# snipsco/sda

Hardware: AMD Instinct MI355X
Metric: share-gen + clerk-sum elements/sec (mod q) (higher is better)
Workload: dtype u64

## Files before the change

include/sda_hip_debug.h:

```cpp
#ifndef SDA_HIP_DEBUG_H
#define SDA_HIP_DEBUG_H
#include <stddef.h>
#ifdef __cplusplus
extern "C" {
#endif
int  sda_debug_hooks_compiled_in(void);
int  sda_debug_set_knob(const char* name, long value);
void sda_debug_reset_knobs(void);
int  sda_debug_env_knobs_compiled_in(void);
const char* sda_debug_last_kernel(void);
const char* sda_debug_last_reveal_kernel(void);
int  sda_debug_stream_create(void** stream);
int  sda_debug_stream_destroy(void* stream);
int  sda_debug_stream_synchronize(void* stream);
int  sda_debug_mem_info(size_t* free_bytes, size_t* total_bytes);
int  sda_debug_poly1305_rows_dev(const unsigned char* keys, const unsigned char* d_msgs, size_t msg_slot,
                                 const unsigned long long* d_msg_bytes, size_t rows, size_t max_msg_bytes, unsigned char* tags);
struct sda_secret_masker;
int  sda_debug_secret_masker_mask_batch_seeded_dev(struct sda_secret_masker* m, const unsigned* seed_words, const long long* d_secrets,
                                                   size_t participants, size_t len, size_t secrets_stride,
                                                   unsigned long long first_participant, long long* d_masks, size_t mask_stride,
                                                   long long* d_masked, size_t masked_stride, void* stream);
int  sda_debug_last_mask_plan(unsigned out[4]);
struct sda_sharing_scheme;
int  sda_debug_select_path(const struct sda_sharing_scheme* scheme, const char* knobs, char* out, size_t cap);
#ifdef __cplusplus
}
#endif
#endif
```

sda_amd/capi.py:

```python
from __future__ import annotations

import ctypes as C
import os

_HERE = os.path.dirname(os.path.abspath(__file__))
RELEASE_LIB_PATH = os.path.join(_HERE, "lib", "libsda_hip.so")
TEST_LIB_PATH = os.path.join(_HERE, "lib", "libsda_hip_test.so")
LIB_PATH = os.environ.get("SDA_HIP_LIBRARY") or RELEASE_LIB_PATH

c_i64p = C.POINTER(C.c_int64)
c_u8p = C.POINTER(C.c_uint8)
c_sizep = C.POINTER(C.c_size_t)
c_i64pp = C.POINTER(c_i64p)
c_voidpp = C.POINTER(C.c_void_p)

OK = 0
ERR_BATCH_INPUT_WRONG_LENGTH = -1
ERR_SHARING_FAILED = -2
ERR_INPUTS_MUST_HAVE_SAME_LENGTH = -3
ERR_NOT_ENOUGH_SHARES = -4
ERR_WRONG_DIMENSION = -5
ERR_MISMATCHING_DIMENSION = -6
ERR_ASSERTION = -7
ERR_INVALID_ARGUMENT = -8
# ... 161 lines not shown
                                                    C.c_size_t, C.c_size_t, C.c_void_p, C.c_size_t, C.c_void_p, C.c_void_p]),
    "sda_share_generator_generate_sealed_rows_dev": (C.c_int, [_H, _H, _H, C.c_char_p, C.c_char_p, C.c_void_p, C.c_size_t, C.c_size_t,
                                                               C.c_size_t, C.c_uint64, C.c_void_p, C.c_size_t, C.c_void_p, C.c_void_p]),
    "sda_share_combiner_update_sealed_rows_dev": (C.c_int, [_H, _H, _H, C.c_char_p, C.c_char_p, C.c_void_p, C.c_size_t,
                                                            C.c_void_p, C.c_size_t, C.c_size_t, C.c_void_p, C.c_void_p,
                                                            C.c_void_p]),
    "sda_share_combiner_finish_sealed_rows_dev": (C.c_int, [_H, _H, _H, C.c_char_p, C.c_char_p, C.c_void_p, C.c_size_t, C.c_void_p,
                                                            C.c_void_p]),
    "sda_mask_combiner_begin_dev": (C.c_int, [_H, C.c_size_t, C.c_void_p]),
    "sda_mask_combiner_update_dev": (C.c_int, [_H, C.c_void_p, C.c_size_t, C.c_size_t, C.c_size_t, C.c_void_p]),
    "sda_mask_combiner_update_sealed_rows_dev": (C.c_int, [_H, _H, _H, C.c_char_p, C.c_char_p, C.c_void_p, C.c_size_t,
                                                           C.c_void_p, C.c_size_t, C.c_size_t, C.c_void_p, C.c_void_p,
                                                           C.c_void_p]),
    "sda_mask_combiner_finish_dev": (C.c_int, [_H, C.c_void_p, C.c_size_t, C.c_void_p]),
    "sda_secret_reconstructor_begin_dev": (C.c_int, [_H, c_sizep, C.c_size_t, C.c_size_t, C.c_void_p]),
    "sda_secret_reconstructor_update_dev": (C.c_int, [_H, C.c_size_t, C.c_void_p, C.c_size_t, C.c_size_t, C.c_void_p]),
    "sda_secret_reconstructor_update_sealed_rows_dev": (C.c_int, [_H, _H, _H, C.c_char_p, C.c_char_p, C.c_size_t, C.c_void_p,
                                                                  C.c_size_t, C.c_void_p, C.c_size_t, C.c_size_t, C.c_void_p,
                                                                  C.c_void_p, C.c_void_p]),
    "sda_secret_reconstructor_finish_dev": (C.c_int, [_H, C.c_void_p, C.c_size_t, C.c_void_p]),
    "sda_comm_unique_id": (C.c_int, [c_u8p]),
    "sda_comm_init": (C.c_int, [c_u8p, C.c_int, C.c_int, _HP]),
    "sda_comm_free": (None, [_H]),
    "sda_comm_rank": (C.c_int, [_H]),
    "sda_comm_world": (C.c_int, [_H]),
    "sda_comm_device": (C.c_int, [_H]),
    "sda_comm_rccl_version": (C.c_int, []),
    "sda_modular_allreduce_dev": (C.c_int, [_H, C.c_int64, C.c_void_p, C.c_size_t, C.c_void_p, C.c_void_p]),
    "sda_modsum_parts_dev": (C.c_int, [C.c_int64, C.c_void_p, C.c_size_t, C.c_size_t, C.c_size_t, C.c_void_p,
                                       C.c_void_p]),
    "sda_fill_synthetic_dev": (C.c_int, [C.c_void_p, C.c_size_t, C.c_size_t, C.c_size_t, C.c_uint64, C.c_uint64,
                                         C.c_int64, C.c_void_p]),
    "sda_event_create": (C.c_int, [c_voidpp]),
    "sda_event_destroy": (C.c_int, [C.c_void_p]),
    "sda_event_record": (C.c_int, [C.c_void_p, C.c_void_p]),
    "sda_event_elapsed_ms": (C.c_int, [C.c_void_p, C.c_void_p, C.POINTER(C.c_float)]),
}

HOOK_SIGNATURES = {
    "sda_debug_set_knob": (C.c_int, [C.c_char_p, C.c_long]),
    "sda_debug_reset_knobs": (None, []),
    "sda_debug_env_knobs_compiled_in": (C.c_int, []),
    "sda_debug_stream_create": (C.c_int, [c_voidpp]),
    "sda_debug_stream_destroy": (C.c_int, [C.c_void_p]),
    "sda_debug_stream_synchronize": (C.c_int, [C.c_void_p]),
    "sda_debug_mem_info": (C.c_int, [c_sizep, c_sizep]),
    "sda_debug_select_path": (C.c_int, [_SS, C.c_char_p, C.c_char_p, C.c_size_t]),
    "sda_debug_last_reveal_kernel": (C.c_char_p, []),
    "sda_debug_poly1305_rows_dev": (C.c_int, [C.c_char_p, C.c_void_p, C.c_size_t, C.c_void_p, C.c_size_t, C.c_size_t, C.c_char_p]),
    "sda_debug_secret_masker_mask_batch_seeded_dev": (C.c_int, [_H, C.c_void_p, C.c_void_p, C.c_size_t, C.c_size_t, C.c_size_t,
                                                                C.c_uint64, C.c_void_p, C.c_size_t, C.c_void_p, C.c_size_t,
                                                                C.c_void_p]),
    "sda_debug_last_mask_plan": (C.c_int, [C.POINTER(C.c_uint * 4)]),
}

_loaded = {}
_active_path = None


def _load_path(path):
    lib = _loaded.get(path)
    if lib is None:
        if not os.path.exists(path):
            raise OSError(f"{path} is missing: build it with __graft_entry__.build(); "
                          "there is no fallback implementation")
        lib = C.CDLL(path)
        for name, (res, args) in SIGNATURES.items():
            fn = getattr(lib, name)
            fn.restype = res
            fn.argtypes = args
        if lib.sda_debug_hooks_compiled_in():
            for name, (res, args) in HOOK_SIGNATURES.items():
                fn = getattr(lib, name)
                fn.restype = res
                fn.argtypes = args
        _loaded[path] = lib
    return lib


class _ActiveLibrary:

    def __getattr__(self, name):
        lib = _load_path(_active_path or LIB_PATH)
        if name in HOOK_SIGNATURES and not lib.sda_debug_hooks_compiled_in():
            raise AttributeError(f"{name} exists only in libsda_hip_test.so: call sda_amd.capi.use_test_hooks() first "
                                 f"(the release library {active_path()} has no test hooks)")
        return getattr(lib, name)


_proxy = _ActiveLibrary()


def load():
    _load_path(_active_path or LIB_PATH)
    return _proxy


def active_path() -> str:
    return _active_path or LIB_PATH


def has_test_hooks() -> bool:
    return bool(_load_path(active_path()).sda_debug_hooks_compiled_in())


def use_test_hooks():
# ... 43 lines not shown
```

sda_amd/csrc/kernels.hpp:

```cpp
#pragma once
#include <stddef.h>
#include <stdint.h>
#include <hip/hip_runtime_api.h>

namespace sda {

struct ModParams {
    uint64_t m;
    uint64_t mu;
    uint64_t lemire_thr;
    uint64_t lemire_thr2;
};

struct MontParams {
    uint64_t p;
    uint64_t pinv;
};

struct DrbgKey {
    uint32_t w[8];
};

#define SDA_MAT_ARG_MAX 448
struct MatArg {
// ... 196 lines not shown
size_t scan_aux_entries(size_t n);
hipError_t launch_scan_u32(const uint32_t* d_in, uint64_t* d_out, size_t n, uint64_t* d_total, uint64_t* d_aux,
                           hipStream_t s);
hipError_t launch_varint_write(const VarintRows& R, const uint64_t* d_block_off, uint8_t* d_out,
                               uint64_t* d_row_offsets, hipStream_t s);
hipError_t launch_varint_count(const uint8_t* d_bytes, size_t n_bytes, uint32_t* d_block_counts, hipStream_t s);
hipError_t launch_varint_decode(const uint8_t* d_bytes, size_t n_bytes, const uint64_t* d_block_val_off,
                                size_t rows, size_t len, size_t row_stride, int64_t* d_out, uint32_t* d_status,
                                hipStream_t s);
struct RowRanges {
    const uint64_t* offsets;
    const uint64_t* lengths;
    uint64_t slot;
};
hipError_t launch_varint_stream_decode(const uint8_t* d_bytes, size_t n_bytes, const RowRanges& rr, size_t rows,
                                       size_t len, size_t row_stride, int64_t* d_out, uint32_t* d_status, hipStream_t s);
hipError_t launch_varint_stream_encode(const VarintRows& R, uint8_t* d_out, size_t slot_bytes, uint64_t* d_row_bytes,
                                       hipStream_t s);
hipError_t launch_varint_stream_combine(const uint8_t* d_bytes, size_t n_bytes, const RowRanges& rr, size_t jobs,
                                        size_t rows_per_job, size_t len, uint64_t* d_acc_lo, int64_t* d_acc_hi,
                                        uint32_t* d_status, hipStream_t s);
struct SboxState;
hipError_t launch_sealed_stream_combine(const uint8_t* d_boxes, size_t slot, const uint64_t* d_row_bytes, size_t rows,
                                        size_t max_box_bytes, const SboxState* d_states, size_t len, uint64_t* d_acc_lo,
                                        int64_t* d_acc_hi, uint32_t* d_status, hipStream_t s, int* waves);
struct WeightedJob {
    const uint64_t* Rt;
    uint32_t k;
    uint64_t batches;
    uint64_t m, mu, pinv;
};
hipError_t launch_sealed_stream_weighted(const uint8_t* d_boxes, size_t slot, const uint64_t* d_row_bytes, size_t rows,
                                         size_t max_box_bytes, const SboxState* d_states, size_t len, size_t first_pos,
                                         const WeightedJob& J, uint64_t* d_acc_lo, int64_t* d_acc_hi, uint32_t* d_status,
                                         hipStream_t s);
hipError_t launch_weighted_rows(const int64_t* d_shares, size_t row_stride, size_t rows, size_t first_pos, const WeightedJob& J,
                                uint64_t* d_acc_lo, int64_t* d_acc_hi, hipStream_t s);
hipError_t launch_transpose_u64(const uint64_t* d_in, uint64_t* d_out, uint32_t k, uint32_t n, hipStream_t s);
hipError_t launch_varint_seal_stream(const VarintRows& R, uint8_t* d_boxes, size_t slot_bytes, const SboxState* d_states,
                                     uint64_t* d_msg_bytes, hipStream_t s);
struct ShareJob {
    const int64_t* secrets;  size_t secrets_stride;
    size_t len, participants;
    uint64_t batches;
    uint64_t first_participant;
    uint32_t n, k, t;
    uint32_t additive;
    uint32_t direct_rows;
    const uint64_t* M;
    ModParams mod;
    MontParams mont;
    DrbgKey key;
};
hipError_t launch_share_seal_stream(const ShareJob& J, int rounds, uint8_t* d_boxes, size_t slot_bytes, const SboxState* d_states,
                                    uint64_t* d_msg_bytes, hipStream_t s);
struct SumRows {
    const uint64_t* acc_lo;  const int64_t* acc_hi;
    size_t jobs, len;
    uint64_t m, mu;
};
size_t sum_seal_blocks(size_t len);
hipError_t launch_sum_lengths(const SumRows& S, uint32_t* d_block_bytes, hipStream_t s);
hipError_t launch_sum_seal_wide(const SumRows& S, const uint64_t* d_block_off, uint8_t* d_boxes, size_t slot_bytes,
                                const SboxState* d_states, uint64_t* d_msg_bytes, hipStream_t s);
hipError_t launch_varint_rowcheck(const uint8_t* d_bytes, size_t n_bytes, const uint64_t* d_offsets, size_t rows,
                                  size_t len, const uint64_t* d_block_val_off, uint32_t* d_status, hipStream_t s);

hipError_t launch_base64_decode_rows(const uint8_t* d_text, const uint64_t* d_offsets, size_t text_slot,
                                     const uint64_t* d_lengths, size_t rows, size_t max_chars, uint8_t* d_out,
                                     size_t out_slot, uint64_t* d_out_bytes, uint32_t* d_status, uint32_t* d_row_status,
                                     hipStream_t s);
hipError_t launch_base64_encode_rows(const uint8_t* d_in, size_t in_slot, const uint64_t* d_in_bytes, size_t rows,
                                     size_t max_bytes, uint8_t* d_text, size_t text_slot, uint64_t* d_text_bytes,
                                     hipStream_t s);

struct SboxState {
    uint32_t subkey[8];
    uint32_t n0, n1;
    uint32_t s[4];
    uint32_t r64[5], rS[5];
    uint32_t bad, pad[7];
    uint32_t rpow[64][5];
};
size_t sbox_regions(size_t max_msg_bytes);
hipError_t launch_sealedbox_open(const uint8_t pk[32], const uint8_t sk[32], const uint8_t* d_boxes, size_t slot,
                                 const uint64_t* d_row_bytes, size_t rows, size_t max_box_bytes, uint8_t* d_out, size_t out_slot,
                                 uint64_t* d_out_bytes, uint32_t* d_ok, uint32_t* d_status, SboxState* d_states,
                                 uint32_t* d_partial, hipStream_t s);
hipError_t launch_sealedbox_verify(const uint8_t pk[32], const uint8_t sk[32], const uint8_t* d_boxes, size_t slot,
                                   const uint64_t* d_row_bytes, size_t rows, size_t max_box_bytes, uint64_t* d_out_bytes,
                                   uint32_t* d_ok, uint32_t* d_status, SboxState* d_states, uint32_t* d_partial, hipStream_t s);
hipError_t launch_sealedbox_seal(const uint8_t* d_esk, const uint8_t* d_pks, size_t n_pks, size_t rows_per_key,
                                 const uint8_t* d_msgs, size_t msg_slot, const uint64_t* d_msg_bytes, size_t rows,
                                 size_t max_msg_bytes, uint8_t* d_boxes, size_t slot, uint64_t* d_row_bytes, SboxState* d_states,
                                 uint32_t* d_partial, hipStream_t s);
hipError_t launch_sealedbox_seal_setup(const uint8_t* d_esk, const uint8_t* d_pks, size_t n_pks, size_t rows_per_key, uint8_t* d_boxes,
                                       size_t slot, size_t rows, SboxState* d_states, hipStream_t s);
hipError_t launch_sealedbox_seal_auth(const uint64_t* d_msg_bytes, size_t rows, size_t max_msg_bytes, uint8_t* d_boxes, size_t slot,
                                      uint64_t* d_row_bytes, SboxState* d_states, uint32_t* d_partial, hipStream_t s);
hipError_t launch_sealedbox_poly_test(const uint8_t* d_keys, const uint8_t* d_msgs, size_t msg_slot, const uint64_t* d_msg_bytes,
                                      size_t rows, size_t max_msg_bytes, uint8_t* d_heads, uint64_t* d_head_bytes,
                                      SboxState* d_states, uint32_t* d_partial, hipStream_t s);

hipError_t launch_modsum_parts(const int64_t* d_parts, size_t parts, size_t part_stride, size_t len,
                               const ModParams& mod, int64_t* d_out, hipStream_t s);
hipError_t launch_fill_synthetic(int64_t* d_out, size_t participants, size_t len, size_t stride,
// ... 5 lines not shown
```

sda_amd/csrc/sda_capi.cpp:

```cpp
#include "../../include/sda_hip.h"

#include <hip/hip_runtime_api.h>
#include <errno.h>
#include <stdarg.h>
#include <stdio.h>
#include <stdlib.h>
#include <atomic>
#include <string.h>
#include <sys/random.h>

#include <algorithm>
#include <new>
#include <string>
#include <vector>

#include "capi_internal.hpp"
#include "host_chacha.hpp"
#include "host_math.hpp"
#include "kernels.hpp"
#include "modarith.hpp"
#include "path_select.hpp"

using namespace sda;

// ... 2540 lines not shown
    if (L == 0) HIP_TRY(launch_varint_stream_decode(d_bytes, rows * slot_bytes, rr, rows, 0, 0, nullptr, d_status, c->ctx.pick(stream)));
    return c->mark_pending(c->ctx.pick(stream));
}

extern "C" int sda_share_combiner_update_sealed_rows_dev(sda_share_combiner_t* c, sda_varint_codec_t* codec, sda_sealedbox_t* b,
                                                         const uint8_t pk[32], const uint8_t sk[32], const uint8_t* d_boxes,
                                                         size_t slot_bytes, const uint64_t* d_row_bytes, size_t rows,
                                                         size_t max_box_bytes, uint32_t* d_ok, uint32_t* d_status, void* stream) {
    if (!c || !codec || !b) return fail(SDA_ERR_INVALID_ARGUMENT, "NULL handle");
    if (!pk || !sk) return fail(SDA_ERR_INVALID_ARGUMENT, "NULL argument");
    if (!c->begun) return fail(SDA_ERR_STATE, "update before begin");
    if (c->acc.rust_signed) return fail(SDA_ERR_UNSUPPORTED, "the wire-fed updates sum in 128 bits: SDA_VALUES_RUST_SIGNED takes decode + update[_dev]");
    if (c->jobs != 1) return fail(SDA_ERR_STATE, "the sealed form feeds ONE job: the combiner was begun with %zu jobs", c->jobs);
    if (rows == 0) return SDA_OK;
    if (!d_status || !d_boxes || !d_row_bytes) return fail(SDA_ERR_INVALID_ARGUMENT, "NULL device pointer");
    if (slot_bytes % 16 || ((uintptr_t)d_boxes & 15u)) return fail(SDA_ERR_INVALID_ARGUMENT, "boxes must be 16-byte aligned (buffer and slot_bytes)");
    if (max_box_bytes > slot_bytes) return fail(SDA_ERR_INVALID_ARGUMENT, "max_box_bytes exceeds slot_bytes");
    SDA_TRY(c->ctx.use());
    hipStream_t s = c->ctx.pick(stream);
    const SboxState* d_states = nullptr;
    SDA_TRY(capi_sealedbox_verify_rows(b, pk, sk, d_boxes, slot_bytes, d_row_bytes, rows, max_box_bytes, d_ok, d_status, c->ctx.device, s,
                                       &d_states));
    SDA_TRY(c->join_pending(s));
    int waves = 0;
    HIP_TRY(launch_sealed_stream_combine(d_boxes, slot_bytes, d_row_bytes, rows, max_box_bytes, d_states, c->dimension,
                                         c->acc.lo.as<uint64_t>(), c->acc.hi.as<int64_t>(), d_status, s, &waves));
    note_kernel("sbox_poly_kernel + sealed_stream_combine_kernel<%d>", waves);
    snprintf(g_last_call_kernels, sizeof g_last_call_kernels, "%s", g_last_gen_kernel);
    return c->mark_pending(s);
}

extern "C" int sda_sealedbox_seal_share_rows_dev(sda_sealedbox_t* b, sda_varint_codec_t* codec, const uint8_t* pks, size_t n_pks,
                                                 size_t rows_per_key, const uint8_t* esk, const int64_t* d_values, size_t rows,
                                                 size_t len, size_t row_stride, uint8_t* d_boxes, size_t slot_bytes,
                                                 uint64_t* d_row_bytes, void* stream) {
    if (!b || !codec) return fail(SDA_ERR_INVALID_ARGUMENT, "NULL handle");
    if (!pks || n_pks == 0 || rows_per_key == 0) return fail(SDA_ERR_INVALID_ARGUMENT, "bad recipient key arguments");
    if (!d_boxes || !d_row_bytes || (len > 0 && !d_values)) return fail(SDA_ERR_INVALID_ARGUMENT, "NULL device pointer");
    if (row_stride < len) return fail(SDA_ERR_INVALID_ARGUMENT, "row_stride < len");
    if (slot_bytes % 16 || ((uintptr_t)d_boxes & 15u)) return fail(SDA_ERR_INVALID_ARGUMENT, "boxes must be 16-byte aligned (buffer and slot_bytes)");
    if (len > (SIZE_MAX - 64) / 10 || slot_bytes < sda_varint_slot_size(len) + SDA_SEALBYTES)
        return fail(SDA_ERR_INVALID_ARGUMENT, "slot_bytes < sda_varint_slot_size(len) + 48");
    if (capi_sealedbox_device(b) != codec->ctx.device)
        return fail(SDA_ERR_INVALID_ARGUMENT, "the sealed-box handle lives on device %d, the codec on device %d", capi_sealedbox_device(b), codec->ctx.device);
    if (rows == 0) return SDA_OK;
    SDA_TRY(codec->ctx.use());
    SDA_TRY(capi_sealedbox_seal_share_rows(b, pks, n_pks, rows_per_key, esk, VarintRows{d_values, rows, len, row_stride}, d_boxes, slot_bytes,
                                           d_row_bytes, codec->ctx.pick(stream)));
    note_kernel("varint_seal_stream_kernel + sbox_poly_kernel");
    snprintf(g_last_call_kernels, sizeof g_last_call_kernels, "%s", g_last_gen_kernel);
    return SDA_OK;
}

extern "C" int sda_share_generator_generate_sealed_rows_dev(sda_share_generator_t* g, sda_varint_codec_t* codec, sda_sealedbox_t* b,
                                                            const uint8_t* pks, const uint8_t* esk, const int64_t* d_secrets,
                                                            size_t participants, size_t len, size_t secrets_stride,
                                                            uint64_t first_participant, uint8_t* d_boxes, size_t slot_bytes,
                                                            uint64_t* d_row_bytes, void* stream) {
    if (!g || !codec || !b) return fail(SDA_ERR_INVALID_ARGUMENT, "NULL handle");
    if (!pks) return fail(SDA_ERR_INVALID_ARGUMENT, "NULL clerk keys");
    if (!d_boxes || !d_row_bytes || (len > 0 && !d_secrets)) return fail(SDA_ERR_INVALID_ARGUMENT, "NULL device pointer");
    if (secrets_stride < len) return fail(SDA_ERR_INVALID_ARGUMENT, "secrets_stride < len");
    if (slot_bytes % 16 || ((uintptr_t)d_boxes & 15u)) return fail(SDA_ERR_INVALID_ARGUMENT, "boxes must be 16-byte aligned (buffer and slot_bytes)");
    const size_t B = (len + g->k - 1) / g->k;
    if (B > (SIZE_MAX - 64) / 10 || slot_bytes < sda_varint_slot_size(B) + SDA_SEALBYTES)
        return fail(SDA_ERR_INVALID_ARGUMENT, "slot_bytes < sda_varint_slot_size(batches) + 48");
    if (capi_sealedbox_device(b) != codec->ctx.device || g->ctx.device != codec->ctx.device)
        return fail(SDA_ERR_INVALID_ARGUMENT, "the generator lives on device %d, the sealed-box handle on device %d, the codec on device %d",
                    g->ctx.device, capi_sealedbox_device(b), codec->ctx.device);
    if (g->rust_signed)
        return fail(SDA_ERR_UNSUPPORTED, "the sealed form computes canonical shares only: SDA_VALUES_RUST_SIGNED takes generate_batch_dev + seal_share_rows_dev");
    if (!g->additive && g->k + g->t > 32)
        return fail(SDA_ERR_UNSUPPORTED, "the sealed form serves packed Shamir with secret_count + privacy_threshold <= 32 (this scheme: %u): "
                                         "call generate_batch_dev + sda_sealedbox_seal_share_rows_dev", g->k + g->t);
    size_t rows = 0;
    if (__builtin_mul_overflow(participants, (size_t)g->n, &rows)) return fail(SDA_ERR_INVALID_ARGUMENT, "participants * share_count overflows");
    if (participants == 0) return SDA_OK;
    SDA_TRY(check_streams(first_participant, participants));
    SDA_TRY(g->ctx.use());
    const bool sys = effective_sys(g);
    if (!g->additive && !g->mseal_loaded) {
        SDA_TRY(g->d_Mseal.reserve((g->Mmont.size() + g->Msys.size()) * 8));
        HIP_TRY(hipMemcpy(g->d_Mseal.p, g->Mmont.data(), g->Mmont.size() * 8, hipMemcpyHostToDevice));
        if (!g->Msys.empty())
            HIP_TRY(hipMemcpy(g->d_Mseal.as<uint64_t>() + g->Mmont.size(), g->Msys.data(), g->Msys.size() * 8, hipMemcpyHostToDevice));
        g->mseal_loaded = true;
    }
    ShareJob J{};
    J.secrets = d_secrets; J.secrets_stride = secrets_stride; J.len = len; J.participants = participants; J.batches = B;
    J.first_participant = first_participant;
    J.n = g->n; J.k = g->k; J.t = g->t; J.additive = g->additive ? 1u : 0u;
    J.direct_rows = sys ? g->t : 0;
    J.M = g->additive ? nullptr : g->d_Mseal.as<uint64_t>() + (sys ? g->Mmont.size() : 0);
    J.mod = g->mod; J.mont = g->mont;
    if (len > 0) J.key = g->drbg.call_key();
    g_last_gen_kernel[0] = 0;
    const int st = capi_sealedbox_seal_generated_rows(b, pks, esk, J, g->drbg.rounds, d_boxes, slot_bytes, d_row_bytes, g->ctx.pick(stream));
    explicit_bzero(&J.key, sizeof J.key);
    if (st != SDA_OK) return st;
    note_kernel("share_seal_stream_kernel<%d> + sbox_poly_kernel", g->drbg.rounds);
    snprintf(g_last_call_kernels, sizeof g_last_call_kernels, "%s", g_last_gen_kernel);
    return SDA_OK;
}

extern "C" int sda_share_combiner_finish_sealed_rows_dev(sda_share_combiner_t* c, sda_varint_codec_t* codec, sda_sealedbox_t* b,
                                                         const uint8_t pk[32], const uint8_t* esk, uint8_t* d_boxes, size_t slot_bytes,
// ... 108 lines not shown
```

sda_amd/csrc/varint_kernels.hip:

```cpp
#include <hip/hip_runtime.h>
#include <stdint.h>

#include "capi_internal.hpp"
#include "drbg_quad.hpp"
#include "kernels.hpp"
#include "modarith.hpp"
#include "sbox_primitives.hpp"

namespace sda {

static constexpr int kVT = 256;
static constexpr int kVals = 8;
static constexpr int kBytes = 16;

__device__ __forceinline__ uint64_t zigzag(int64_t v) { return ((uint64_t)v << 1) ^ (uint64_t)(v >> 63); }
__device__ __forceinline__ uint32_t varint_len(uint64_t zz) {
    const uint32_t x = (64u - (uint32_t)__clzll(zz | 1ull)) + 6u;
    return (x * 37u) >> 8;
}

__device__ __forceinline__ uint32_t block_exscan(uint32_t v, uint32_t* lds_waves, uint32_t* total) {
    const int lane = threadIdx.x & 63, wave = threadIdx.x >> 6;
    uint32_t incl = v;
#pragma unroll
// ... 986 lines not shown
            x = (int64_t)s0; y = (int64_t)s1;
            return;
        }
        U128 a0{0, 0}, a1{0, 0};
        uint32_t since = 0;
        const uint64_t e0 = b0 * J.k, e1 = e0 + J.k;
        for (uint32_t i = 0; i < J.k; ++i) {
            const uint64_t v0 = e0 + i < J.len ? canon_i64(sp[e0 + i], m, mu) : 0;
            const uint64_t v1 = e1 + i < J.len ? canon_i64(sp[e1 + i], m, mu) : 0;
            const uint64_t cf = row[i];
            mac128(a0, cf, v0);
            mac128(a1, cf, v1);
            if (++since == 4) { mont_acc_condsub(a0, J.mont.p); mont_acc_condsub(a1, J.mont.p); since = 0; }
        }
        for (uint32_t i = 0; i < T; ++i) {
            drbg_pair<ROUNDS>(J.key, qc, stream, pair, T, i, J.mod, r0, r1);
            const uint64_t cf = row[J.k + i];
            mac128(a0, cf, r0);
            mac128(a1, cf, r1);
            if (++since == 4) { mont_acc_condsub(a0, J.mont.p); mont_acc_condsub(a1, J.mont.p); since = 0; }
        }
        mont_acc_condsub(a0, J.mont.p);
        mont_acc_condsub(a1, J.mont.p);
        x = (int64_t)mont_redc(a0, J.mont.p, J.mont.pinv);
        y = (int64_t)mont_redc(a1, J.mont.p, J.mont.pinv);
    }
};

template <int ROUNDS>
__global__ __launch_bounds__(kStreamWaves * 64) void share_seal_stream_kernel(ShareJob J, uint32_t by_rows, uint8_t* __restrict__ boxes,
                                                                              uint64_t slot, const SboxState* __restrict__ states,
                                                                              uint64_t* __restrict__ msg_bytes) {
    __shared__ __attribute__((aligned(16))) uint8_t tiles[kStreamWaves][kEncTile];
    __shared__ uint32_t kstream[kStreamWaves][kKsTile];
    const int wave = __builtin_amdgcn_readfirstlane(threadIdx.x >> 6);
    uint64_t c, p;
    if (by_rows) {
        const uint64_t r = (uint64_t)blockIdx.x * kStreamWaves + wave;
        c = r / J.participants; p = r - c * J.participants;
    } else {
        const uint32_t groups = (J.n + kStreamWaves - 1) / kStreamWaves;
        p = blockIdx.x / groups;
        c = (uint64_t)(blockIdx.x - p * groups) * kStreamWaves + wave;
    }
    if (c >= J.n || p >= J.participants) return;
    const uint64_t r = c * J.participants + p;
    if (states[r].bad) { if ((threadIdx.x & 63) == 0) msg_bytes[r] = 0; return; }
    EncXSalsa crypt;
    crypt.open(states[r], kstream[wave]);
    ShareValues<ROUNDS> vals(J, (uint32_t)c, p);
    encode_row(vals, J.batches, r, boxes + r * slot + 48, tiles[wave], msg_bytes, crypt);
}

static constexpr int kSumVals = kVT * kVals;
static constexpr int kSumStage = 64 + kSumVals * 10;
static constexpr int kSumKsBlocks = kSumStage / 64;
static constexpr int kSumKsStride = 17;

size_t sum_seal_blocks(size_t len) { return (size_t)((len + kSumVals - 1) / kSumVals); }

__global__ __launch_bounds__(kVT) void sum_len_kernel(SumRows S, uint32_t* __restrict__ block_bytes) {
    __shared__ uint32_t waves[kVT / 64];
    const uint64_t job = blockIdx.y;
    const uint64_t* lo = S.acc_lo + job * S.len;
    const int64_t* hi = S.acc_hi + job * S.len;
    const uint64_t i0 = (uint64_t)blockIdx.x * kSumVals + threadIdx.x;
    uint32_t sum = 0;
    for (int u = 0; u < kVals; ++u) {
        const uint64_t i = i0 + (uint64_t)u * kVT;
        if (i < S.len) sum += varint_len(zigzag((int64_t)mod_i128(lo[i], hi[i], S.m, S.mu)));
    }
    uint32_t total;
    (void)block_exscan(sum, waves, &total);
    if (threadIdx.x == 0) block_bytes[job * gridDim.x + blockIdx.x] = total;
}

__global__ __launch_bounds__(kVT) void sum_seal_wide_kernel(SumRows S, const uint64_t* __restrict__ block_off, uint8_t* __restrict__ boxes,
                                                            uint64_t slot, const SboxState* __restrict__ states,
                                                            uint64_t* __restrict__ msg_bytes) {
    __shared__ uint32_t waves[kVT / 64];
    __shared__ __attribute__((aligned(16))) uint8_t stage[kSumStage + 16];
    __shared__ uint32_t ks[kSumKsBlocks * kSumKsStride];
    const uint64_t job = blockIdx.y, blk = blockIdx.x, n_blk = gridDim.x;
    const bool last = blk + 1 == n_blk;
    const SboxState& st = states[job];
    if (st.bad) { if (last && threadIdx.x == 0) msg_bytes[job] = 0; return; }
    const uint64_t off = block_off[job * n_blk + blk] - block_off[job * n_blk];
    const uint32_t pad = (uint32_t)((off + 32) & 63u);
    const uint64_t ks0 = (off + 32) >> 6;
    const uint64_t* lo = S.acc_lo + job * S.len;
    const int64_t* hi = S.acc_hi + job * S.len;
    const uint64_t i0 = blk * kSumVals + (uint64_t)threadIdx.x * kVals;
    uint64_t zz[kVals];
    uint32_t ln[kVals];
    uint32_t sum = 0;
    for (int k = 0; k < kVals; ++k) {
        zz[k] = 0; ln[k] = 0;
        if (i0 + k < S.len) {
            zz[k] = zigzag((int64_t)mod_i128(lo[i0 + k], hi[i0 + k], S.m, S.mu));
            ln[k] = varint_len(zz[k]);
            sum += ln[k];
        }
    }
    uint32_t total;
    uint32_t pos = pad + block_exscan(sum, waves, &total);
#pragma unroll
// ... 92 lines not shown
                                       size_t len, size_t row_stride, int64_t* d_out, uint32_t* d_status, hipStream_t s) {
    if (rows == 0) return hipSuccess;
    varint_stream_decode_kernel<<<dim3((unsigned)vceil(rows, kStreamWaves)), dim3(kStreamWaves * 64), 0, s>>>(
        d_bytes, n_bytes, d_offsets, rows, len, row_stride, d_out, d_status);
    return hipGetLastError();
}

hipError_t launch_varint_stream_encode(const VarintRows& R, uint8_t* d_out, size_t slot_bytes, uint64_t* d_row_bytes,
                                       hipStream_t s) {
    if (R.rows == 0) return hipSuccess;
    varint_stream_encode_kernel<<<dim3((unsigned)vceil(R.rows, kStreamWaves)), dim3(kStreamWaves * 64), residency_pad_bytes(knob(KNOB_WIRE_WG_PER_CU), 8192), s>>>(
        R, d_out, slot_bytes, d_row_bytes);
    return hipGetLastError();
}

hipError_t launch_varint_seal_stream(const VarintRows& R, uint8_t* d_boxes, size_t slot_bytes, const SboxState* d_states,
                                     uint64_t* d_msg_bytes, hipStream_t s) {
    if (R.rows == 0) return hipSuccess;
    const uint64_t groups = vceil(R.rows, kStreamWaves);
    if (groups > 0x7FFFFFFFull) return hipErrorInvalidConfiguration;
    varint_seal_stream_kernel<<<dim3((unsigned)groups), dim3(kStreamWaves * 64), 0, s>>>(R, d_boxes, slot_bytes, d_states, d_msg_bytes);
    return hipGetLastError();
}

static bool sum_grid(const SumRows& S, dim3* grid) {
    const uint64_t nb = sum_seal_blocks(S.len);
    if (S.jobs > 65535 || nb * S.jobs > 0xFFFFFFFFull / kVT) return false;
    *grid = dim3((unsigned)nb, (unsigned)S.jobs);
    return true;
}

hipError_t launch_sum_lengths(const SumRows& S, uint32_t* d_block_bytes, hipStream_t s) {
    if (S.jobs == 0 || S.len == 0) return hipSuccess;
    dim3 grid;
    if (!sum_grid(S, &grid)) return hipErrorInvalidConfiguration;
    sum_len_kernel<<<grid, dim3(kVT), 0, s>>>(S, d_block_bytes);
    return hipGetLastError();
}

hipError_t launch_sum_seal_wide(const SumRows& S, const uint64_t* d_block_off, uint8_t* d_boxes, size_t slot_bytes,
                                const SboxState* d_states, uint64_t* d_msg_bytes, hipStream_t s) {
    if (S.jobs == 0) return hipSuccess;
    if (S.len == 0) return hipMemsetAsync(d_msg_bytes, 0, S.jobs * sizeof(uint64_t), s);
    dim3 grid;
    if (!sum_grid(S, &grid)) return hipErrorInvalidConfiguration;
    sum_seal_wide_kernel<<<grid, dim3(kVT), 0, s>>>(S, d_block_off, d_boxes, slot_bytes, d_states, d_msg_bytes);
    return hipGetLastError();
}

hipError_t launch_share_seal_stream(const ShareJob& J, int rounds, uint8_t* d_boxes, size_t slot_bytes, const SboxState* d_states,
                                    uint64_t* d_msg_bytes, hipStream_t s) {
    if (J.participants == 0 || J.n == 0) return hipSuccess;
    const bool by_rows = knob(KNOB_GENSEAL_BY_ROWS) != 0;
    const uint64_t groups = by_rows ? vceil((uint64_t)J.n * J.participants, kStreamWaves) : vceil(J.n, kStreamWaves) * (uint64_t)J.participants;
    if (groups > 0x7FFFFFFFull) return hipErrorInvalidConfiguration;
    const dim3 grid((unsigned)groups), block(kStreamWaves * 64);
    switch (rounds) {
        case 20: share_seal_stream_kernel<20><<<grid, block, 0, s>>>(J, by_rows, d_boxes, slot_bytes, d_states, d_msg_bytes); break;
        case 12: share_seal_stream_kernel<12><<<grid, block, 0, s>>>(J, by_rows, d_boxes, slot_bytes, d_states, d_msg_bytes); break;
        case 8: share_seal_stream_kernel<8><<<grid, block, 0, s>>>(J, by_rows, d_boxes, slot_bytes, d_states, d_msg_bytes); break;
        default: return hipErrorInvalidValue;
    }
    return hipGetLastError();
}

hipError_t launch_varint_stream_combine(const uint8_t* d_bytes, size_t n_bytes, const RowRanges& d_offsets, size_t jobs,
                                        size_t rows_per_job, size_t len, uint64_t* d_acc_lo, int64_t* d_acc_hi,
                                        uint32_t* d_status, hipStream_t s) {
    if (jobs == 0 || rows_per_job == 0 || len == 0) return hipSuccess;
    const bool wide = vceil(rows_per_job, 16) * jobs >= 512;
    const uint64_t groups = vceil(rows_per_job, wide ? 16 : 8);
    if (groups * jobs > 0x7FFFFFFFull) return hipErrorInvalidConfiguration;
    if (wide)
        varint_stream_combine_kernel<16><<<dim3((unsigned)(groups * jobs)), dim3(16 * 64), residency_pad_bytes(knob(KNOB_WIRE_WG_PER_CU), 49152), s>>>(
            d_bytes, n_bytes, d_offsets, rows_per_job, groups, len, d_acc_lo, d_acc_hi, d_status);
    else
        varint_stream_combine_kernel<8><<<dim3((unsigned)(groups * jobs)), dim3(8 * 64), 0, s>>>(
            d_bytes, n_bytes, d_offsets, rows_per_job, groups, len, d_acc_lo, d_acc_hi, d_status);
    return hipGetLastError();
}

hipError_t launch_sealed_stream_combine(const uint8_t* d_boxes, size_t slot, const uint64_t* d_row_bytes, size_t rows,
                                        size_t max_box_bytes, const SboxState* d_states, size_t len, uint64_t* d_acc_lo,
                                        int64_t* d_acc_hi, uint32_t* d_status, hipStream_t s, int* waves) {
    if (waves) *waves = 0;
    if (rows == 0) return hipSuccess;
    const bool wide = knob(KNOB_SEALED_WAVES) == 16;
    const uint64_t groups = vceil(rows, wide ? 16 : 8);
    if (groups > 0x7FFFFFFFull) return hipErrorInvalidConfiguration;
    if (waves) *waves = wide ? 16 : 8;
    if (wide)
        sealed_stream_combine_kernel<16><<<dim3((unsigned)groups), dim3(16 * 64), 0, s>>>(d_boxes, slot, d_row_bytes, max_box_bytes, d_states,
                                                                                       rows, len, d_acc_lo, d_acc_hi, d_status);
    else
        sealed_stream_combine_kernel<8><<<dim3((unsigned)groups), dim3(8 * 64), 0, s>>>(d_boxes, slot, d_row_bytes, max_box_bytes, d_states,
                                                                                     rows, len, d_acc_lo, d_acc_hi, d_status);
    return hipGetLastError();
}

hipError_t launch_sealed_stream_weighted(const uint8_t* d_boxes, size_t slot, const uint64_t* d_row_bytes, size_t rows,
                                         size_t max_box_bytes, const SboxState* d_states, size_t len, size_t first_pos,
                                         const WeightedJob& J, uint64_t* d_acc_lo, int64_t* d_acc_hi, uint32_t* d_status,
                                         hipStream_t s) {
    if (rows == 0) return hipSuccess;
    const uint64_t groups = vceil(rows, 8);
    if (groups > 0x7FFFFFFFull) return hipErrorInvalidConfiguration;
// ... 41 lines not shown
```

Before: 118.4 billion.

## Share DRBG draws and secrets across clerk waves via LDS staging in share-seal kernel

Result: no change. 118.4 billion, median of 6 (+0.0%).

```diff
diff --git a/include/sda_hip_debug.h b/include/sda_hip_debug.h
--- a/include/sda_hip_debug.h
+++ b/include/sda_hip_debug.h
@@ -22,6 +22,7 @@
                                                    unsigned long long first_participant, long long* d_masks, size_t mask_stride,
                                                    long long* d_masked, size_t masked_stride, void* stream);
 int  sda_debug_last_mask_plan(unsigned out[4]);
+int  sda_debug_genseal_geometry(unsigned share_count, unsigned secret_count, unsigned privacy_threshold, int additive, unsigned out[6]);
 struct sda_sharing_scheme;
 int  sda_debug_select_path(const struct sda_sharing_scheme* scheme, const char* knobs, char* out, size_t cap);
 #ifdef __cplusplus
diff --git a/sda_amd/capi.py b/sda_amd/capi.py
--- a/sda_amd/capi.py
+++ b/sda_amd/capi.py
@@ -237,6 +237,7 @@
                                                                 C.c_uint64, C.c_void_p, C.c_size_t, C.c_void_p, C.c_size_t,
                                                                 C.c_void_p]),
     "sda_debug_last_mask_plan": (C.c_int, [C.POINTER(C.c_uint * 4)]),
+    "sda_debug_genseal_geometry": (C.c_int, [C.c_uint, C.c_uint, C.c_uint, C.c_int, C.POINTER(C.c_uint * 6)]),
 }
 
 _loaded = {}
diff --git a/sda_amd/csrc/kernels.hpp b/sda_amd/csrc/kernels.hpp
--- a/sda_amd/csrc/kernels.hpp
+++ b/sda_amd/csrc/kernels.hpp
@@ -272,6 +272,8 @@
     MontParams mont;
     DrbgKey key;
 };
+struct GensealGeometry { uint32_t shared, waves, groups, steps, terms, lds_bytes; };
+GensealGeometry genseal_geometry(uint32_t n, uint32_t kt, uint32_t additive);
 hipError_t launch_share_seal_stream(const ShareJob& J, int rounds, uint8_t* d_boxes, size_t slot_bytes, const SboxState* d_states,
                                     uint64_t* d_msg_bytes, hipStream_t s);
 struct SumRows {
diff --git a/sda_amd/csrc/sda_capi.cpp b/sda_amd/csrc/sda_capi.cpp
--- a/sda_amd/csrc/sda_capi.cpp
+++ b/sda_amd/csrc/sda_capi.cpp
@@ -2616,6 +2616,17 @@
     return SDA_OK;
 }
 
+#ifdef SDA_TEST_HOOKS
+extern "C" int sda_debug_genseal_geometry(unsigned share_count, unsigned secret_count, unsigned privacy_threshold, int additive,
+                                          unsigned out[6]) {
+    if (!out) return fail(SDA_ERR_INVALID_ARGUMENT, "out is NULL");
+    if (share_count == 0) return fail(SDA_ERR_INVALID_ARGUMENT, "share_count is 0");
+    const GensealGeometry G = genseal_geometry(share_count, secret_count + privacy_threshold, additive ? 1u : 0u);
+    out[0] = G.shared; out[1] = G.waves; out[2] = G.groups; out[3] = G.steps; out[4] = G.terms; out[5] = G.lds_bytes;
+    return SDA_OK;
+}
+#endif
+
 extern "C" int sda_share_generator_generate_sealed_rows_dev(sda_share_generator_t* g, sda_varint_codec_t* codec, sda_sealedbox_t* b,
                                                             const uint8_t* pks, const uint8_t* esk, const int64_t* d_secrets,
                                                             size_t participants, size_t len, size_t secrets_stride,
diff --git a/sda_amd/csrc/varint_kernels.hip b/sda_amd/csrc/varint_kernels.hip
--- a/sda_amd/csrc/varint_kernels.hip
+++ b/sda_amd/csrc/varint_kernels.hip
@@ -1062,6 +1062,161 @@
     encode_row(vals, J.batches, r, boxes + r * slot + 48, tiles[wave], msg_bytes, crypt);
 }
 
+static constexpr int kShareWaves = 8;
+static constexpr uint32_t kShareWaveLds = kEncTile + 4 * kKsTile;
+static constexpr uint32_t kShareLdsBudget = 80 * 1024;
+
+GensealGeometry genseal_geometry(uint32_t n, uint32_t kt, uint32_t additive) {
+    GensealGeometry g{};
+    if (n == 0) return g;
+    g.terms = additive ? n : kt;
+    g.groups = (n + kShareWaves - 1) / kShareWaves;
+    g.waves = (n + g.groups - 1) / g.groups;
+    const uint32_t left = kShareLdsBudget - g.waves * kShareWaveLds, step = g.terms * kEncVals * 8;
+    g.steps = step == 0 ? 0 : left / step < 8 ? left / step : 8;
+    g.lds_bytes = g.waves * kShareWaveLds + g.steps * step;
+    g.shared = g.steps >= 1;
+    return g;
+}
+
+template <int ROUNDS>
+struct SharedShareValues {
+    static constexpr int kDepth = 1;
+    const ShareJob& J;
+    const int64_t* __restrict__ sp;
+    const uint64_t* __restrict__ row;
+    uint64_t* stage;
+    uint64_t stream, n_steps;
+    uint32_t S, terms, units_per_step, first_draw, wave, waves, phase;
+    uint32_t T, own;
+    bool secret_last;
+    QuadCol qc;
+    __device__ __forceinline__ SharedShareValues(const ShareJob& J_, uint64_t* stage_, uint32_t S_, uint32_t terms_, uint32_t c0,
+                                                 uint32_t size, uint32_t c, uint64_t p, uint32_t wave_, uint32_t waves_)
+        : J(J_), stage(stage_), S(S_), terms(terms_), wave(wave_), waves(waves_), phase(0) {
+        sp = J.secrets + p * J.secrets_stride;
+        stream = J.first_participant + p;
+        qc = quad_col(J.key);
+        n_steps = (J.batches + kEncVals - 1) / kEncVals;
+        T = J.additive ? J.n - 1 : J.t;
+        const uint32_t direct = J.additive ? J.n - 1 : J.direct_rows;
+        row = J.additive || c < direct ? nullptr : J.M + (uint64_t)(c - direct) * (J.k + J.t);
+        if (J.additive) {
+            secret_last = c0 + size == J.n;
+            units_per_step = secret_last ? J.n : size;
+            first_draw = secret_last ? 0 : c0;
+            own = c < direct ? c - first_draw : terms;
+        } else {
+            secret_last = false;
+            units_per_step = J.k + J.t;
+            first_draw = 0;
+            own = c < direct ? J.k + c : terms;
+        }
+    }
+    __device__ __forceinline__ uint64_t* slot(uint32_t s, uint32_t term) const {
+        return stage + ((s * terms + term) * (uint32_t)kEncVals + 2u * (threadIdx.x & 63u));
+    }
+    __device__ __forceinline__ void begin_block(uint64_t j0) {
+        __syncthreads();
+        const uint64_t left = n_steps - j0;
+        const uint32_t steps = left < S ? (uint32_t)left : S;
+        const uint32_t units = steps * units_per_step;
+        const uint64_t m = J.mod.m, mu = J.mod.mu;
+        uint32_t s = 0, term = wave;
+        for (uint32_t u = wave; u < units; u += waves, term += waves) {
+            while (term >= units_per_step) { term -= units_per_step; ++s; }
+            const uint64_t pair = (j0 + s) * (kEncVals / 2) + (threadIdx.x & 63u);
+            const uint64_t b0 = 2 * pair;
+            uint64_t v0, v1;
+            if (J.additive) {
+                if (secret_last && term == J.n - 1) {
+                    v0 = b0 < J.len ? canon_i64(sp[b0], m, mu) : 0;
+                    v1 = b0 + 1 < J.len ? canon_i64(sp[b0 + 1], m, mu) : 0;
+                } else {
+                    drbg_pair<ROUNDS>(J.key, qc, stream, pair, T, first_draw + term, J.mod, v0, v1);
+                }
+            } else if (term < J.k) {
+                const uint64_t e0 = b0 * J.k + term, e1 = e0 + J.k;
+                v0 = e0 < J.len ? canon_i64(sp[e0], m, mu) : 0;
+                v1 = e1 < J.len ? canon_i64(sp[e1], m, mu) : 0;
+            } else {
+                drbg_pair<ROUNDS>(J.key, qc, stream, pair, T, term - J.k, J.mod, v0, v1);
+            }
+            uint64_t* q = slot(s, term);
+            q[0] = v0; q[1] = v1;
+        }
+        __syncthreads();
+    }
+    __device__ __forceinline__ void idle() {
+        for (uint64_t j0 = 0; j0 < n_steps; j0 += S) begin_block(j0);
+    }
+    __device__ __forceinline__ void get(int, uint64_t j, int64_t& x, int64_t& y) {
+        const uint32_t s = phase;
+        if (s == 0) begin_block(j);
+        phase = s + 1 == S ? 0 : s + 1;
+        if (own < terms) {
+            const uint64_t* q = slot(s, own);
+            x = (int64_t)q[0]; y = (int64_t)q[1];
+            return;
+        }
+        if (J.additive) {
+            const uint64_t m = J.mod.m;
+            const uint64_t* q = slot(s, J.n - 1);
+            uint64_t s0 = q[0], s1 = q[1];
+            for (uint32_t i = 0; i < T; ++i) {
+                q = slot(s, i);
+                s0 = submod(s0, q[0], m);
+                s1 = submod(s1, q[1], m);
+            }
+            x = (int64_t)s0; y = (int64_t)s1;
+            return;
+        }
+        U128 a0{0, 0}, a1{0, 0};
+        uint32_t since = 0;
+        const uint32_t kt = J.k + J.t;
+        for (uint32_t i = 0; i < kt; ++i) {
+            const uint64_t* q = slot(s, i);
+            const uint64_t cf = row[i];
+            mac128(a0, cf, q[0]);
+            mac128(a1, cf, q[1]);
+            if (++since == 4) { mont_acc_condsub(a0, J.mont.p); mont_acc_condsub(a1, J.mont.p); since = 0; }
+        }
+        mont_acc_condsub(a0, J.mont.p);
+        mont_acc_condsub(a1, J.mont.p);
+        x = (int64_t)mont_redc(a0, J.mont.p, J.mont.pinv);
+        y = (int64_t)mont_redc(a1, J.mont.p, J.mont.pinv);
+    }
+};
+
+template <int ROUNDS>
+__global__ __launch_bounds__(kShareWaves * 64) void share_seal_stream_shared_kernel(ShareJob J, uint32_t groups, uint32_t S, uint32_t terms,
+                                                                                     uint8_t* __restrict__ boxes, uint64_t slot,
+                                                                                     const SboxState* __restrict__ states,
+                                                                                     uint64_t* __restrict__ msg_bytes) {
+    extern __shared__ __attribute__((aligned(16))) uint8_t share_lds[];
+    const uint32_t wave = __builtin_amdgcn_readfirstlane(threadIdx.x >> 6), waves = blockDim.x >> 6;
+    uint8_t* tile = share_lds + (size_t)wave * kShareWaveLds;
+    uint32_t* kstream = reinterpret_cast<uint32_t*>(tile + kEncTile);
+    uint64_t* stage = reinterpret_cast<uint64_t*>(share_lds + (size_t)waves * kShareWaveLds);
+    const uint64_t p = blockIdx.x / groups;
+    const uint32_t q = (uint32_t)(blockIdx.x - p * groups);
+    const uint32_t base = J.n / groups, rem = J.n - base * groups;
+    const uint32_t size = base + (q < rem ? 1u : 0u), c0 = q * base + (q < rem ? q : rem);
+    const uint32_t c = c0 + wave;
+    const bool clerk = wave < size;
+    const uint64_t r = (uint64_t)(clerk ? c : c0) * J.participants + p;
+    SharedShareValues<ROUNDS> vals(J, stage, S, terms, c0, size, c, p, wave, waves);
+    const bool bad = clerk && states[r].bad;
+    if (!clerk || bad) {
+        if (bad && (threadIdx.x & 63) == 0) msg_bytes[r] = 0;
+        vals.idle();
+        return;
+    }
+    EncXSalsa crypt;
+    crypt.open(states[r], kstream);
+    encode_row(vals, J.batches, r, boxes + r * slot + 48, tile, msg_bytes, crypt);
+}
+
 static constexpr int kSumVals = kVT * kVals;
 static constexpr int kSumStage = 64 + kSumVals * 10;
 static constexpr int kSumKsBlocks = kSumStage / 64;
@@ -1260,6 +1415,17 @@
                                     uint64_t* d_msg_bytes, hipStream_t s) {
     if (J.participants == 0 || J.n == 0) return hipSuccess;
     const bool by_rows = knob(KNOB_GENSEAL_BY_ROWS) != 0;
+    const GensealGeometry G = genseal_geometry(J.n, J.k + J.t, J.additive);
+    if (!by_rows && G.shared) {
+        const uint64_t wgs = (uint64_t)G.groups * J.participants;
+        if (wgs > 0x7FFFFFFFull) return hipErrorInvalidConfiguration;
+        if (rounds != 20 && rounds != 12 && rounds != 8) return hipErrorInvalidValue;
+        auto kern = rounds == 20 ? share_seal_stream_shared_kernel<20> : rounds == 12 ? share_seal_stream_shared_kernel<12> : share_seal_stream_shared_kernel<8>;
+        if (G.lds_bytes > 64 * 1024)
+            if (hipError_t e = hipFuncSetAttribute(reinterpret_cast<const void*>(kern), hipFuncAttributeMaxDynamicSharedMemorySize, (int)G.lds_bytes)) return e;
+        kern<<<dim3((unsigned)wgs), dim3(G.waves * 64), G.lds_bytes, s>>>(J, G.groups, G.steps, G.terms, d_boxes, slot_bytes, d_states, d_msg_bytes);
+        return hipGetLastError();
+    }
     const uint64_t groups = by_rows ? vceil((uint64_t)J.n * J.participants, kStreamWaves) : vceil(J.n, kStreamWaves) * (uint64_t)J.participants;
     if (groups > 0x7FFFFFFFull) return hipErrorInvalidConfiguration;
     const dim3 grid((unsigned)groups), block(kStreamWaves * 64);
```
